# piyanon108/iGate4xSoftphoneDSP

Hardware: AMD Instinct MI355X
Metric: Msamples/s G.711 decode+RMS, 65536ch@8kHz; %HBM roofline at 1/2/4/8 GPU (higher is better)
Workload: dtype u8

## Files before the change

igate4xsoftphonedsp_amd/csrc/igdsp_capi.hip:

```cpp
#include "igdsp_ctx.h"
#include "igdsp_txstage.h"

#include <algorithm>
#include <atomic>
#include <chrono>
#include <cmath>
#include <cstdio>
#include <cstdlib>
#include <cstring>
#include <mutex>
#include <new>
#include <string>
#include <unordered_map>
#include <vector>

using namespace igdsp;
using igdsp_rx::kSlot;
using igdsp_rx::kStageDepth;

struct igdsp_ctx::TxSide {
    igdsp_tx::Stager st;
    hipStream_t stream = nullptr;
    hipEvent_t ev[4] = {};
    igdsp_tx_chan *d_state = nullptr;
// ... 146 lines not shown
    for (int i = 0; i < igdsp_rx::RingMem::kArrays; ++i) if (*ctx->ring.array(i)) (void)hipHostFree(*ctx->ring.array(i));
    const igdsp_rx::Published &p0 = ctx->pub.set(0), &p1 = ctx->pub.set(1);
    void *hosts[] = {ctx->h_up, p0.last, p0.hold, p0.probe, p1.last, p1.hold, p1.probe};
    for (void *p : hosts) if (p) (void)hipHostFree(p);
    void *devs[] = {ctx->d_up, ctx->d_stats, ctx->d_last, ctx->d_hold, ctx->d_probe, ctx->d_queues, ctx->d_enc_tab[0], ctx->d_enc_tab[1]};
    for (void *p : devs) if (p) (void)hipFree(p);
    delete ctx;
    return IGDSP_OK;
}

const char *igdsp_last_error(const igdsp_ctx *ctx) { return ctx ? ctx->err.c_str() : ""; }

int igdsp_device_info(const igdsp_ctx *ctx, int *device, int *compute_units, char *name, size_t name_len)
{
    if (!ctx) return IGDSP_EINVAL;
    if (device) *device = ctx->device;
    if (compute_units) *compute_units = ctx->cus;
    if (name && name_len) { std::strncpy(name, ctx->name.c_str(), name_len - 1); name[name_len - 1] = 0; }
    return IGDSP_OK;
}

int igdsp_set_variant(igdsp_ctx *ctx, int variant)
{
    if (!ctx || variant < 0 || variant > 4) return IGDSP_EINVAL;
    ctx->variant = variant;
    return IGDSP_OK;
}

static uint32_t lookup(igdsp_ctx *ctx, int32_t call_id)
{
    if (call_id >= 0 && call_id < kDirectCalls) return ctx->direct[(size_t)call_id].load(std::memory_order_acquire);
    std::lock_guard<std::mutex> g(ctx->far_mu);
    auto it = ctx->far.find(call_id);
    return it == ctx->far.end() ? kNoChan : it->second;
}

int igdsp_map_call(igdsp_ctx *ctx, int32_t call_id, uint32_t channel)
{
    if (!ctx) return IGDSP_EINVAL;
    if (channel >= ctx->max_channels) return IGDSP_ERANGE;
    if (call_id >= 0 && call_id < kDirectCalls) ctx->direct[(size_t)call_id].store(channel, std::memory_order_release);
    else { std::lock_guard<std::mutex> g(ctx->far_mu); ctx->far[call_id] = channel; }
    return IGDSP_OK;
}

int igdsp_unmap_call(igdsp_ctx *ctx, int32_t call_id)
{
// ... 1034 lines not shown
    if (!ctx || !d_src || !d_dst || (stride & 3u) || n_seg == 0 || (groups && n_items % groups)) return IGDSP_EINVAL;
    HIP_TRY(ctx, hipSetDevice(ctx->device));
    HIP_TRY(ctx, launch_stream_walk(cfg_of(ctx, pick(ctx, stream)), d_src, n_items, stride, hdr, groups, n_seg, trickle, d_dst, d_dst2, pick(ctx, stream)));
    return IGDSP_OK;
}

int igdsp_internal_stream_mix(igdsp_ctx *ctx, const void *d_src, void *d_dst, uint32_t n_items, int r, int w, int waves, void *stream)
{
    if (!ctx || !d_src || !d_dst || (reinterpret_cast<uintptr_t>(d_src) & 3u) || (reinterpret_cast<uintptr_t>(d_dst) & 15u)) return IGDSP_EINVAL;
    HIP_TRY(ctx, hipSetDevice(ctx->device));
    HIP_TRY(ctx, launch_stream_mix(cfg_of(ctx, pick(ctx, stream)), d_src, d_dst, n_items, r, w, waves, pick(ctx, stream)));
    return IGDSP_OK;
}

int igdsp_internal_stream_mix2(igdsp_ctx *ctx, const void *d_src, void *d_dst, void *d_dst2, uint32_t n_items, int r, int w, int waves, void *stream,
                               const void *d_src2)
{
    if (!ctx || !d_src || !d_dst || !d_dst2 || (reinterpret_cast<uintptr_t>(d_src2) & 15u) || ((reinterpret_cast<uintptr_t>(d_src) | reinterpret_cast<uintptr_t>(d_dst) | reinterpret_cast<uintptr_t>(d_dst2)) & 15u)) return IGDSP_EINVAL;
    HIP_TRY(ctx, hipSetDevice(ctx->device));
    HIP_TRY(ctx, launch_stream_mix(cfg_of(ctx, pick(ctx, stream)), d_src, d_dst, n_items, r, w, waves, pick(ctx, stream), d_dst2, d_src2));
    return IGDSP_OK;
}

int igdsp_internal_diag_chunk32(igdsp_ctx *ctx, const uint8_t *d_payload, const uint8_t *d_codec, uint32_t C, uint32_t F,
                                igdsp_frame_stats *d_stats, uint64_t *d_diag, void *stream)
{
    if (!ctx || !d_payload || !d_codec || !d_stats || !d_diag || C < 32) return IGDSP_EINVAL;
    HIP_TRY(ctx, hipSetDevice(ctx->device));
    HIP_TRY(ctx, launch_diag_chunk32(cfg_of(ctx, pick(ctx, stream)), d_payload, d_codec, C, F, d_stats, d_diag, pick(ctx, stream)));
    return IGDSP_OK;
}

int igdsp_dev_alloc(igdsp_ctx *ctx, void **d_ptr, size_t bytes)
{
    if (!ctx || !d_ptr) return IGDSP_EINVAL;
    *d_ptr = nullptr;
    if (bytes == 0) return IGDSP_OK;
    if (hipSetDevice(ctx->device) != hipSuccess) return IGDSP_ENODEV;
    hipError_t e = hipMalloc(d_ptr, bytes);
    return e == hipSuccess ? IGDSP_OK : fail(ctx, IGDSP_ENOMEM, "hipMalloc", e);
}

int igdsp_dev_free(igdsp_ctx *ctx, void *d_ptr)
{
    if (!ctx) return IGDSP_EINVAL;
    if (!d_ptr) return IGDSP_OK;
// ... 128 lines not shown
```

igate4xsoftphonedsp_amd/csrc/igdsp_device.h:

```cpp
#pragma once
#include "igdsp_internal.h"

#include <algorithm>
#include <cstdlib>

namespace igdsp {

__device__ __forceinline__ uint32_t ulaw_abs(uint32_t code)
{
    const uint32_t u = ~code & 0x7Fu;
    return ((((u & 15u) * 2u + 33u) << (u >> 4)) - 33u) << 2;
}

__device__ __forceinline__ uint32_t alaw_abs(uint32_t code)
{
    const uint32_t a = (code ^ 0x55u) & 0x7Fu;
    const uint32_t s = a >> 4, q = a & 15u;
    const uint32_t m = (s == 0u) ? (q * 2u + 1u) : ((q * 2u + 33u) << (s - 1u));
    return m << 3;
}

typedef uint32_t u32x4_t __attribute__((ext_vector_type(4)));
__device__ __forceinline__ uint4 ld_stream(const uint4 *p)
{
// ... 322 lines not shown
    return b >= nb ? b : ((b & 1u) ? half + (b >> 1) : (b >> 1));
}

template <int W>
struct BlockQueue { uint32_t next, batch[8], tag[8]; };

template <int W>
__device__ __forceinline__ void bq_init(BlockQueue<W> &q, uint32_t *gq, uint32_t G, uint32_t gb1)
{
    q.next = (uint32_t)W;
    for (int i = 0; i < 8; ++i) q.tag[i] = 0xFFFFFFFFu;
    q.batch[0] = blockIdx.x; q.tag[0] = 0u;
    q.batch[1] = gq ? gb1 + G : blockIdx.x + G; q.tag[1] = 1u;
}

template <int W>
__device__ __forceinline__ uint32_t bq_grab(BlockQueue<W> &q, uint32_t *gq, uint32_t G, uint32_t lane, uint32_t nb)
{
    uint32_t v = 0;
    if (lane == 0) {
        const uint32_t s = atomicAdd(&q.next, 1u);
        const uint32_t j = s / (uint32_t)W, w = s - j * (uint32_t)W;
        if (w == 0u) {
            const uint32_t nb = gq ? atomicAdd(gq, 1u) + G : blockIdx.x + (j + 1u) * G;
            __hip_atomic_store(&q.batch[(j + 1u) & 7u], nb, __ATOMIC_RELAXED, __HIP_MEMORY_SCOPE_WORKGROUP);
            __hip_atomic_store(&q.tag[(j + 1u) & 7u], j + 1u, __ATOMIC_RELEASE, __HIP_MEMORY_SCOPE_WORKGROUP);
        }
        while (__hip_atomic_load(&q.tag[j & 7u], __ATOMIC_ACQUIRE, __HIP_MEMORY_SCOPE_WORKGROUP) != j)
            __builtin_amdgcn_s_sleep(2);
        v = spread_batch(__hip_atomic_load(&q.batch[j & 7u], __ATOMIC_RELAXED, __HIP_MEMORY_SCOPE_WORKGROUP), nb) * (uint32_t)W + w;
    }
    return (uint32_t)__builtin_amdgcn_readfirstlane((int)v);
}

__device__ __forceinline__ void bq_finish(uint32_t *gq, uint32_t G)
{
    if (gq == nullptr) return;
    __syncthreads();
    if (threadIdx.x == 0 && atomicAdd(gq + 1, 1u) == G - 1u) { gq[0] = 0u; gq[1] = 0u; }
}


struct EncK { int k_and, k_add, sh; uint32_t c_shift, c_seg, base; };

template <int VARIANT>
__device__ __forceinline__ EncK enc_consts(bool alaw)
{
    EncK k;
    if (VARIANT == IGDSP_ENC_SUN16) {
        k.k_and = alaw ? -8 : 0; k.k_add = alaw ? 0 : 0x84; k.sh = 0;
        k.c_shift = alaw ? 23u : 24u;
        k.c_seg = 24u;
    } else {
        k.k_and = alaw ? 0 : 1; k.k_add = alaw ? 0 : 0x21; k.sh = alaw ? 3 : 2;
        k.c_shift = 26u;
        k.c_seg = alaw ? 27u : 26u;
    }
    k.base = alaw ? 0xD5u : 0xFFu;
    return k;
}

template <int VARIANT>
// ... 68 lines not shown
```

igate4xsoftphonedsp_amd/csrc/igdsp_internal.h:

```cpp
#pragma once
#include <hip/hip_runtime.h>
#include <stdint.h>
#include "igdsp.h"
#include "igdsp_route.h"

namespace igdsp {

struct LaunchCfg {
    int compute_units;
    uint32_t *gqueue;
    bool out_spread = false;
    const uint8_t *enc_tab = nullptr;
};

struct WinArgs {
    uint4 *work = nullptr;
    uint32_t gate_mask = 0, alarm = IGDSP_PROBE_ALARM, n_seg = 1, n_groups = 0, F = 0;
    uint32_t gpb = 0, gsh = 0;
    igdsp_chan_hold *hold = nullptr;
    const uint8_t *gate = nullptr;
    igdsp_chan_probe *probe = nullptr;
};
constexpr int kWinRing = 16;
constexpr int kWinBlkCh = 256;
// ... 48 lines not shown
hipError_t launch_conf_copy_ab(const LaunchCfg &cfg, const uint8_t *g711, const uint8_t *codec, const int16_t *pcm, const uint16_t *len,
                               const uint16_t *gain, const uint32_t *port_ptr, const uint32_t *members, uint32_t n_members, uint32_t C, uint32_t P,
                               uint32_t F, uint32_t n, int16_t *out, igdsp_frame_stats *stats, hipStream_t s);
hipError_t launch_bss_select(const LaunchCfg &cfg, const igdsp_rtp_info *info, const uint8_t *g711, const uint8_t *codec, const int16_t *pcm,
                             const uint16_t *len, const uint16_t *gain, const uint32_t *group_ptr, const uint32_t *members, uint32_t n_members,
                             const uint8_t *mute, uint32_t C, uint32_t G, uint32_t F, uint32_t n, uint32_t vote_frames, igdsp_bss_state *state,
                             uint32_t *words, int32_t *sel, int16_t *out, igdsp_frame_stats *stats, hipStream_t s);
hipError_t launch_bss_copy_ab(const LaunchCfg &cfg, const igdsp_rtp_info *info, const uint8_t *g711, const uint8_t *codec, const int16_t *pcm,
                              const uint16_t *len, const uint16_t *gain, const uint32_t *group_ptr, const uint32_t *members, uint32_t n_members,
                              const uint8_t *mute, uint32_t C, uint32_t G, uint32_t F, uint32_t n, uint32_t vote_frames, igdsp_bss_state *state,
                              uint32_t *words, int32_t *sel, int16_t *out, igdsp_frame_stats *stats, hipStream_t s);
hipError_t launch_jb_receive(const LaunchCfg &cfg, const uint8_t *packets, const uint16_t *sizes, const uint8_t *radio, const uint32_t *arrival,
                             uint32_t C, uint32_t T, uint32_t S, uint32_t stride, uint32_t n, uint32_t delay, igdsp_jb_state *state, void *ring,
                             uint8_t *payload, uint16_t *len, igdsp_rtp_info *info, uint8_t *tick, uint8_t *pkt, hipStream_t s);
hipError_t launch_jb_copy(const LaunchCfg &cfg, const uint8_t *packets, const uint16_t *sizes, const uint8_t *radio, const uint32_t *arrival,
                          uint32_t C, uint32_t T, uint32_t S, uint32_t stride, uint32_t n, uint32_t delay, igdsp_jb_state *state, void *ring,
                          uint8_t *payload, uint16_t *len, igdsp_rtp_info *info, uint8_t *tick, uint8_t *pkt, hipStream_t s);
hipError_t launch_wav_expand(const LaunchCfg &cfg, const uint8_t *payload, uint32_t C, uint32_t F, uint32_t n, uint32_t rate,
                             uint8_t *files, uint64_t file_stride, hipStream_t s);
hipError_t launch_g726(const LaunchCfg &cfg, const uint8_t *in, uint8_t *out, uint64_t n_bytes, int mode, hipStream_t s);
hipError_t launch_gen_uniform(uint8_t *out, uint64_t n_bytes, uint64_t seed, uint64_t first_byte, hipStream_t s);
hipError_t launch_stream_rw(const LaunchCfg &cfg, const void *src, size_t bytes, void *dst, hipStream_t s);
hipError_t launch_stream_cluster(const LaunchCfg &cfg, const void *src, size_t bytes, void *dst, int k, hipStream_t s);
hipError_t launch_stream_pieces(const LaunchCfg &cfg, const void *src, uint32_t n_items, uint32_t stride, uint32_t hdr, int mode, int rows, void *dst, void *dst2, hipStream_t s);
hipError_t launch_stream_walk(const LaunchCfg &cfg, const void *src, uint32_t n_items, uint32_t stride, uint32_t hdr, uint32_t groups, uint32_t n_seg,
                              uint32_t trickle, void *dst, void *dst2, hipStream_t s);
hipError_t launch_stream_mix(const LaunchCfg &cfg, const void *src, void *dst, uint32_t n_items, int r, int w, int waves, hipStream_t s, void *dst2 = nullptr, const void *src2 = nullptr);
hipError_t launch_stream_read(const LaunchCfg &cfg, const void *src, size_t bytes, uint64_t *sink, hipStream_t s);

}
```

igate4xsoftphonedsp_amd/csrc/igdsp_k_meter.hip:

```cpp
#include "igdsp_device.h"

namespace igdsp {

__global__ __launch_bounds__(256) void k_meter_wave_per_frame(
    const uint8_t *__restrict__ payload, const uint8_t *__restrict__ codec, const uint16_t *__restrict__ len,
    uint32_t C, uint32_t first_frame, uint32_t n_frames, uint32_t n, igdsp_frame_stats *__restrict__ stats,
    int16_t *__restrict__ pcm, igdsp_aggregate *agg, uint32_t rank)
{
    __shared__ int16_t lut[2][256];
    __shared__ uint2 agg_slots[4 * 4];
    for (uint32_t i = threadIdx.x; i < 512u; i += 256u) {
        const uint32_t code = i & 255u;
        const int ax = (int)((i >> 8) ? alaw_abs(code) : ulaw_abs(code));
        lut[i >> 8][code] = (int16_t)((code & 0x80u) ? ax : -ax);
    }
    __syncthreads();

    const uint32_t lane = threadIdx.x & 63u, wave = threadIdx.x >> 6;
    const bool dword_ok = ((n & 3u) == 0u) && ((reinterpret_cast<uintptr_t>(payload) & 3u) == 0u) &&
                          ((reinterpret_cast<uintptr_t>(pcm) & 7u) == 0u);
    uint64_t a_sumsq = 0, a_samples = 0;
    uint32_t a_frames = 0, a_sil = 0, a_clip = 0, a_bm = 0, a_peak = 0;

    auto load_frame = [&](uint32_t fi) -> uint32_t {
// ... 54 lines not shown
            if (l == 0u) {
                st.sumsq = 0; st.rms = 0.f; st.peak = 0; st.byte_mean = 0; st.flags = IGDSP_FLAG_EMPTY;
            } else {
                st = make_stats(s64, peak, bsum, l, alaw, probe);
                a_sumsq += s64; a_samples += l; a_frames += 1; a_sil += (st.flags & IGDSP_FLAG_SILENT) ? 1u : 0u;
                a_clip += (st.flags & IGDSP_FLAG_CLIPPED) ? 1u : 0u; a_bm += st.byte_mean; a_peak = max(a_peak, peak);
            }
            stats[fi] = st;
        }
    };
    constexpr uint32_t U = 8;
    const uint32_t last = n_frames - 1u;
    for (uint32_t f0 = first_frame + (blockIdx.x * 4u + wave) * U; f0 < n_frames; f0 += gridDim.x * 4u * U) {
        uint32_t w[U];
#pragma unroll
        for (uint32_t u = 0; u < U; ++u) w[u] = load_frame(min(f0 + u, last));
#pragma unroll
        for (uint32_t u = 0; u < U; ++u)
            if (f0 + u < n_frames) process_frame(f0 + u, w[u]);
    }
    if (agg != nullptr) agg_commit_block(agg, rank, agg_slots, 4u, a_sumsq, a_samples, a_frames, a_sil, a_clip, a_bm, a_peak);
}

template <bool STORE_PCM>
__device__ __forceinline__ void process_half(const uint2 *lut, uint2 *strip_half, uint4 (&d)[kLoadsPerChunk],
                                             const uint32_t am, const uint32_t (&fr)[kLoadsPerChunk], const uint32_t (&pm)[kLoadsPerChunk],
                                             const uint32_t off, const uint32_t lane, uint4 *pcm_half, const uint4 *refill,
                                             uint4 *xpose = nullptr)
{
    uint2 e[2][8];
    uint32_t wa[2], wb[2];
    auto issue = [&](int u) {
        const int j = u >> 1, k = u & 1;
        wa[k] = (u & 1) ? d[j].z : d[j].x;
        wb[k] = (u & 1) ? d[j].w : d[j].y;
        const uint32_t lmj = (uint32_t)__builtin_amdgcn_sbfe(am, fr[j], 1) & 0x80808080u;
        const uint32_t ta = (wa[k] & 0x7F7F7F7Fu) | lmj, tb = (wb[k] & 0x7F7F7F7Fu) | lmj;
        e[k][0] = lut_at(lut, ta, off, 0x0C0C0400u); e[k][1] = lut_at(lut, ta, off, 0x0C0C0500u);
        e[k][2] = lut_at(lut, ta, off, 0x0C0C0600u); e[k][3] = lut_at(lut, ta, off, 0x0C0C0700u);
        e[k][4] = lut_at(lut, tb, off, 0x0C0C0400u); e[k][5] = lut_at(lut, tb, off, 0x0C0C0500u);
        e[k][6] = lut_at(lut, tb, off, 0x0C0C0600u); e[k][7] = lut_at(lut, tb, off, 0x0C0C0700u);
    };
    uint32_t sum = 0, peak = 0, bsum = 0;
    uint32_t o[8];
    issue(0);
#pragma unroll
    for (int u = 0; u < 2 * kLoadsPerChunk; ++u) {
        const int j = u >> 1, k = u & 1;
        if (u + 1 < 2 * kLoadsPerChunk) issue(u + 1);
        __builtin_amdgcn_sched_barrier(0);
        bsum = __builtin_amdgcn_sad_u8(wa[k], 0u, bsum);
        bsum = __builtin_amdgcn_sad_u8(wb[k], 0u, bsum);
        sum = sum + e[k][0].x + e[k][1].x; sum = sum + e[k][2].x + e[k][3].x;
        sum = sum + e[k][4].x + e[k][5].x; sum = sum + e[k][6].x + e[k][7].x;
        peak = max(max(peak, e[k][0].y), e[k][1].y); peak = max(max(peak, e[k][2].y), e[k][3].y);
        peak = max(max(peak, e[k][4].y), e[k][5].y); peak = max(max(peak, e[k][6].y), e[k][7].y);
        if (STORE_PCM) {
            o[4 * k + 0] = pack_pcm(wa[k], 0, e[k][0].y, e[k][1].y); o[4 * k + 1] = pack_pcm(wa[k], 2, e[k][2].y, e[k][3].y);
            o[4 * k + 2] = pack_pcm(wb[k], 0, e[k][4].y, e[k][5].y); o[4 * k + 3] = pack_pcm(wb[k], 2, e[k][6].y, e[k][7].y);
        }
        if (k == 1) {
            strip_half[j * 64 + lane] = make_uint2(sum, peak | (bsum << 16) | probe_fail(d[j], pm[j]));
            if (STORE_PCM) {
                const uint32_t wsw = (lane >> 2) & 1u, rsw = lane ^ ((lane >> 3) & 1u);
                xpose[(2u * lane) ^ wsw] = make_uint4(o[0], o[1], o[2], o[3]);
                xpose[(2u * lane + 1u) ^ wsw] = make_uint4(o[4], o[5], o[6], o[7]);
                wave_lds_fence();
                const uint4 v0 = xpose[rsw], v1 = xpose[64u + rsw];
                wave_lds_fence();
                uint4 *op = pcm_half + ((uint32_t)j * 128u + lane);
                op[0] = v0;
                op[64] = v1;
            }
            d[j] = ld_stream(refill + j * 64);
            sum = 0; peak = 0; bsum = 0;
        }
    }
}


template <bool STORE_PCM, bool AGG, bool DIAG = false>
__global__ __launch_bounds__(ChunkGeom<STORE_PCM>::kWaves * 64) void k_meter_chunk64(
    const uint8_t *__restrict__ payload, const uint8_t *__restrict__ codec, uint32_t C, uint32_t n_frames,
    igdsp_frame_stats *__restrict__ stats, int16_t *__restrict__ pcm, igdsp_aggregate *agg, uint32_t rank,
    uint64_t *__restrict__ diag = nullptr, uint32_t *__restrict__ gqueue = nullptr)
{
    constexpr int kWaves = ChunkGeom<STORE_PCM>::kWaves;
    __shared__ uint2 lds[kLutEntries + kWaves * kStripEntries + (STORE_PCM ? kWaves * 256 : 0)];
    constexpr int kRing = 8;
    __shared__ uint32_t q_next, q_batch[kRing], q_tag[kRing];
    __shared__ AggBlock aggb;
    uint64_t d_t0 = 0, d_t1 = 0, d_iter = 0, d_rt0 = 0, d_setup = 0, d_px = 0, d_py = 0, d_red = 0;
    if (DIAG) { d_t0 = now_cycles(); d_rt0 = __builtin_amdgcn_s_memrealtime(); }
    const uint32_t G = gridDim.x;
    uint32_t gb1 = 0;
    if (threadIdx.x == 0 && gqueue != nullptr) gb1 = atomicAdd(gqueue, 1u);
    fill_lut(lds);
    if (threadIdx.x == 0) {
        q_next = kWaves;
        agg_block_init(aggb);
        for (int i = 0; i < kRing; ++i) q_tag[i] = 0xFFFFFFFFu;
        q_batch[0] = blockIdx.x; q_tag[0] = 0u;
        q_batch[1] = gqueue ? gb1 + G : blockIdx.x + G; q_tag[1] = 1u;
    }
    __syncthreads();
    if (DIAG) d_t1 = now_cycles();

    const uint32_t lane = threadIdx.x & 63u, wave = threadIdx.x >> 6;
// ... 87 lines not shown
                if (AGG) {
                    a_sumsq += s << 4; a_bm += bm; a_peak = max(a_peak, peak);
                    u_frames += (uint32_t)kSuperFrames;
                    u_sil += (uint32_t)__builtin_popcountll(__ballot((fl & IGDSP_FLAG_SILENT) != 0u));
                    u_clip += (uint32_t)__builtin_popcountll(__ballot((fl & IGDSP_FLAG_CLIPPED) != 0u));
                }
            }
            wave_lds_fence();
            if (DIAG) { d_iter += 1; d_setup += d_b - d_a; d_px += d_c - d_b; d_py += d_d - d_c; d_red += now_cycles() - d_d; }
            if (!has_next) break;
            sidx = s_next;
            s_next = s_after;
            cur_pt = nxt_pt;
        }
    }
    if (DIAG && lane == 0 && diag != nullptr) {
        uint64_t *o = diag + (uint64_t)(blockIdx.x * kWaves + wave) * 12u;
        o[0] = d_t0; o[1] = d_t1; o[2] = now_cycles(); o[3] = d_setup; o[4] = d_px; o[5] = d_iter; o[6] = d_py;
        o[7] = __builtin_amdgcn_s_getreg((4 << 11) | (0 << 6) | 20);
        o[8] = d_rt0; o[9] = __builtin_amdgcn_s_memrealtime(); o[10] = d_red; o[11] = wave;
    }
    wave_exit(AGG ? agg : nullptr, rank, aggb, (uint32_t)kWaves, lane, gqueue, G, a_sumsq, lane == 0u ? (uint64_t)u_frames * kFrame : 0ull,
              a_bm, a_peak, u_frames, u_sil, u_clip);
}

constexpr int kFatDepth = 4;

template <bool AGG>
__global__ __launch_bounds__(kFatWaves * 64) void k_meter_fat(
    const uint8_t *__restrict__ payload, const uint8_t *__restrict__ codec, uint32_t C, uint32_t n_frames,
    igdsp_frame_stats *__restrict__ stats, igdsp_aggregate *agg, uint32_t rank)
{
    __shared__ uint2 lds[kLutEntries + kFatWaves * kStripEntries];
    fill_lut(lds);
    __syncthreads();

    const uint32_t lane = threadIdx.x & 63u, wave = threadIdx.x >> 6;
    uint2 *strip = lds + kLutEntries + wave * kStripEntries;
    const uint32_t off = (lane & 31u) * 8u;
    uint32_t fr[kLoadsPerChunk], pm[kLoadsPerChunk];
#pragma unroll
    for (int j = 0; j < kLoadsPerChunk; ++j) {
        const uint32_t p = (uint32_t)j * 64u + lane;
        fr[j] = p / 10u;
        pm[j] = probe_mask(p - fr[j] * 10u);
    }
// ... 593 lines not shown
                         reinterpret_cast<const void *>(&k_meter_image<true, false>), reinterpret_cast<const void *>(&k_meter_image<false, false>)};
    for (const void *f : fns) {
        const hipError_t e = hipFuncSetAttribute(f, hipFuncAttributeMaxDynamicSharedMemorySize, lim);
        if (e != hipSuccess) return e;
    }
    return hipSuccess;
}

hipError_t launch_decode_meter(const LaunchCfg &cfg, int variant, const uint8_t *payload, const uint8_t *codec,
                               const uint16_t *len, uint32_t C, uint32_t F, uint32_t n, igdsp_frame_stats *stats,
                               int16_t *pcm, igdsp_aggregate *agg, uint32_t rank, hipStream_t s)
{
    const MeterRoute r = decode_meter_route(C, F, n, variant, len != nullptr, reinterpret_cast<uintptr_t>(payload), reinterpret_cast<uintptr_t>(pcm),
                                            reinterpret_cast<uintptr_t>(stats), (uint32_t)cfg.compute_units, knobs_from_env());
    uint32_t *gq = cfg.gqueue;
    uint64_t *nodiag = nullptr;
    const dim3 g(r.grid), b(r.threads);
    const uint32_t done = r.done, n_frames = C * F;
    with_bool(agg != nullptr, [&](auto A) {
        switch (r.fast) {
        case MeterFast::none: break;
        case MeterFast::fat: hipLaunchKernelGGL((k_meter_fat<A>), g, b, 0, s, payload, codec, C, done, stats, agg, rank); break;
        case MeterFast::chunk:
            with_bool(r.store, [&](auto P) { hipLaunchKernelGGL((k_meter_chunk64<P, A>), g, b, 0, s, payload, codec, C, done, stats, pcm, agg, rank, nodiag, gq); });
            break;
        case MeterFast::tiny:
            with_key(Keys<4, 5, 6, 7, 8>{}, r.key, [&](auto N4) { hipLaunchKernelGGL((k_meter_tiny<N4, A>), g, b, 0, s, payload, codec, C, done, stats, agg, rank, gq); });
            break;
        case MeterFast::strided: {
            auto launch = [&](auto K, auto P) {
                hipLaunchKernelGGL((k_meter_strided<key_q(K), key_tail(K), A, P>), g, b, 0, s, payload, codec, C, done, n, stats, agg, rank, gq, pcm);
            };
            if (r.store) with_key(ReferenceSizeKeys{}, r.key, [&](auto K) { launch(K, std::true_type{}); });
            else         with_key(MeterStridedKeys{}, r.key, [&](auto K) { launch(K, std::false_type{}); });
            break;
        }
        }
    });
    if (r.fast != MeterFast::none) { hipError_t e = hipGetLastError(); if (e != hipSuccess) return e; }
    const dim3 rg(r.rest_grid), rb(r.rest_threads);
    if (r.rest == MeterRest::image) {
        with_bool(agg != nullptr, [&](auto A) { with_bool(len != nullptr, [&](auto L) {
            hipLaunchKernelGGL((k_meter_image<A, L>), rg, rb, r.rest_lds, s, payload, codec, len, C, done, n_frames, n, stats, agg, rank);
        }); });
    } else if (r.rest == MeterRest::wave_per_frame) {
        hipLaunchKernelGGL(k_meter_wave_per_frame, rg, rb, 0, s, payload, codec, len, C, done, n_frames, n, stats, pcm, agg, rank);
    }
// ... 17 lines not shown
```

igate4xsoftphonedsp_amd/csrc/igdsp_k_misc.hip:

```cpp
#include "igdsp_device.h"

namespace igdsp {

constexpr int kWavTile = 16;

__device__ __forceinline__ void wav_header_words(uint32_t (&h)[11], uint32_t rate, uint32_t data_bytes)
{
    h[0] = 0x46464952u;
    h[1] = 36u + data_bytes;
    h[2] = 0x45564157u;
    h[3] = 0x20746D66u;
    h[4] = 16u;
    h[5] = 0x0007u | (2u << 16);
    h[6] = rate;
    h[7] = rate * 4u;
    h[8] = 4u | (16u << 16);
    h[9] = 0x61746164u;
    h[10] = data_bytes;
}

typedef uint32_t u32x4_st4_t __attribute__((ext_vector_type(4), aligned(4)));

__global__ __launch_bounds__(256) void k_wav_expand16(const uint8_t *__restrict__ payload, uint32_t C, uint32_t F, uint32_t n,
                                                      uint32_t rate, uint8_t *__restrict__ files, uint64_t file_stride)
// ... 281 lines not shown
template <int K>
__global__ __launch_bounds__(kBlockThreads) void k_stream_cluster(const uint4 *__restrict__ src, uint32_t n_super, uint4 *__restrict__ dst)
{
    const uint32_t lane = threadIdx.x & 63u, wave = threadIdx.x >> 6;
    const uint32_t n_items = n_super / (uint32_t)K;
    for (uint32_t b = blockIdx.x; b * kWavesPerBlock + wave < n_items; b += gridDim.x) {
        const uint32_t item = b * kWavesPerBlock + wave;
        uint4 acc[K];
#pragma unroll
        for (int k = 0; k < K; ++k) {
            const uint4 *p = src + (((uint64_t)item * (uint32_t)K + (uint32_t)k) * 640u + lane);
            uint4 v[10];
#pragma unroll
            for (int j = 0; j < 10; ++j) v[j] = ld_stream(p + j * 64);
            acc[k] = make_uint4(0, 0, 0, 0);
#pragma unroll
            for (int j = 0; j < 10; ++j) { acc[k].x ^= v[j].x; acc[k].y ^= v[j].y; acc[k].z ^= v[j].z; acc[k].w ^= v[j].w; }
        }
#pragma unroll
        for (int k = 0; k < K; ++k) dst[((uint64_t)item * (uint32_t)K + (uint32_t)k) * 64u + lane] = acc[k];
    }
}

hipError_t launch_stream_cluster(const LaunchCfg &cfg, const void *src, size_t bytes, void *dst, int k, hipStream_t s)
{
    const uint32_t n_super = (uint32_t)(bytes / 10240u);
    const dim3 g(cfg.compute_units), b(kBlockThreads);
    const uint4 *sp = reinterpret_cast<const uint4 *>(src);
    uint4 *dp = reinterpret_cast<uint4 *>(dst);
    if (k == 1) hipLaunchKernelGGL((k_stream_cluster<1>), g, b, 0, s, sp, n_super, dp);
    else if (k == 2) hipLaunchKernelGGL((k_stream_cluster<2>), g, b, 0, s, sp, n_super, dp);
    else if (k == 4) hipLaunchKernelGGL((k_stream_cluster<4>), g, b, 0, s, sp, n_super, dp);
    else if (k == 8) hipLaunchKernelGGL((k_stream_cluster<8>), g, b, 0, s, sp, n_super, dp);
    else if (k == 16) hipLaunchKernelGGL((k_stream_cluster<16>), g, b, 0, s, sp, n_super, dp);
    else return hipErrorInvalidValue;
    return hipGetLastError();
}

hipError_t launch_gen_uniform(uint8_t *out, uint64_t n_bytes, uint64_t seed, uint64_t first_byte, hipStream_t s)
{
    if (n_bytes == 0) return hipSuccess;
    const uint64_t words = (n_bytes >> 3) + 2;
    hipLaunchKernelGGL(k_gen_uniform, dim3(blocks_for(words, 256, 8192)), dim3(256), 0, s, out, n_bytes, seed, first_byte);
    return hipGetLastError();
}

// ... 119 lines not shown
```

igate4xsoftphonedsp_amd/csrc/igdsp_route.h:

```cpp
#pragma once
#include <algorithm>
#include <cstdint>
#include <cstdlib>
#include <optional>
#include <type_traits>
#include <utility>

#include "igdsp.h"

namespace igdsp {


constexpr int kFrame = IGDSP_SAMPLES_PER_FRAME;
constexpr int kChunkFrames = 32;
constexpr int kChunkBytes = kChunkFrames * kFrame;
constexpr int kPiecesPerFrame = kFrame / 16;
constexpr int kPiecesPerChunk = kChunkFrames * kPiecesPerFrame;
constexpr int kLoadsPerChunk = kPiecesPerChunk / 64;
constexpr int kWavesPerBlock = 16;
constexpr int kBlockThreads = kWavesPerBlock * 64;
constexpr int kSuperFrames = 2 * kChunkFrames;
constexpr int kLutEntries = 256 * 32;
constexpr uint32_t kWinMaxSeg = 8;

#ifndef IGDSP_STORE_WAVES
#define IGDSP_STORE_WAVES 4
#endif
template <bool STORE_PCM> struct ChunkGeom { static constexpr int kWaves = STORE_PCM ? IGDSP_STORE_WAVES : kWavesPerBlock; };
constexpr int kFatWaves = 8;
constexpr uint32_t kImgMaxWaves = 12;
#ifndef IGDSP_SSTORE_WAVES
#define IGDSP_SSTORE_WAVES 0
#endif
constexpr int strided_meter_waves(int qp, bool store) { return store ? (IGDSP_SSTORE_WAVES ? IGDSP_SSTORE_WAVES : (qp <= 2 ? 16 : 6)) : (qp <= 11 ? 16 : 12); }
template <int QP, bool STORE = false> struct StridedGeom { static constexpr int kWaves = strided_meter_waves(QP, STORE); };
constexpr int kTinyWaves = 16, kTinyDepth = 4;
#ifndef IGDSP_TINY_SLOT
#define IGDSP_TINY_SLOT 4
#endif
constexpr uint32_t kTinySlot = IGDSP_TINY_SLOT;

#ifndef IGDSP_ENC_WAVES
#define IGDSP_ENC_WAVES 10
#endif
constexpr int kEncWaves = IGDSP_ENC_WAVES;
#ifndef IGDSP_RT_WAVES
#define IGDSP_RT_WAVES 12
#endif
constexpr int kRtWaves = IGDSP_RT_WAVES;
#ifndef IGDSP_RTL_WAVES
#define IGDSP_RTL_WAVES 12
// ... 58 lines not shown
inline uint32_t groups_per_block(uint32_t n_groups, uint32_t cus, std::optional<int> force)
{
    uint32_t gpb = 1u;
    for (uint32_t g = 4u; g > 1u; g >>= 1) if (n_groups % g == 0u && n_groups / g >= cus) { gpb = g; break; }
    if (force) { const uint32_t g = (uint32_t)*force; if ((g == 1u || g == 2u || g == 4u) && n_groups % g == 0u) gpb = g; }
    return gpb;
}
inline uint32_t gpb_shift(uint32_t gpb) { return gpb == 4u ? 2u : (gpb == 2u ? 1u : 0u); }
inline uint32_t rounds_of(uint32_t blocks, uint32_t cus) { return (blocks + cus - 1u) / cus; }

inline bool roundtrip_block_fills(uint32_t blocks, uint32_t cus) { return rounds_of(blocks, cus) == 1u && blocks * 10u >= cus * 6u; }

inline bool window_block_fills(uint32_t blocks, uint32_t cus)
{
    const uint32_t rounds = rounds_of(blocks, cus);
    return rounds == 1u || (uint64_t)blocks * 100u >= (uint64_t)rounds * cus * 85u;
}

enum class MeterFast { none, fat, chunk, tiny, strided };
enum class MeterRest { none, image, wave_per_frame };
struct MeterRoute {
    MeterFast fast = MeterFast::none;
    bool store = false;
    int key = 0;
    uint32_t grid = 0, threads = 0;
    uint32_t done = 0;
    MeterRest rest = MeterRest::none;
    uint32_t rest_grid = 0, rest_threads = 0, rest_lds = 0;
};

inline MeterRoute decode_meter_route(uint32_t C, uint32_t F, uint32_t n, int variant, bool has_len, uintptr_t payload, uintptr_t pcm,
                                     uintptr_t stats, uint32_t cus, const Knobs &k)
{
    MeterRoute r;
    if ((uint64_t)C * F == 0) return r;
    const uint32_t n_frames = C * F;
    const bool chunk_ok = n == (uint32_t)kFrame && !has_len && aligned(payload, 16) && aligned(pcm, 16) && aligned(stats, 16);
    const uint32_t n_super = n_frames / kSuperFrames, whole = n_super * kSuperFrames;
    if (variant == 3 && chunk_ok && pcm == 0 && n_frames >= (uint32_t)kSuperFrames) {
        r.fast = MeterFast::fat;
        r.grid = blocks_for(n_super, kFatWaves, cus); r.threads = kFatWaves * 64; r.done = whole;
    } else if (variant != 1 && chunk_ok && n_frames >= (uint32_t)kSuperFrames) {
        const int w = pcm ? ChunkGeom<true>::kWaves : ChunkGeom<false>::kWaves;
        r.fast = MeterFast::chunk; r.store = pcm != 0;
        r.grid = blocks_for(n_super, w, cus); r.threads = w * 64; r.done = whole;
    }
    if (r.done == 0 && variant != 1 && !has_len && pcm == 0 && (n & 3u) == 0u && n >= 16u && n <= 32u && n_frames >= (uint32_t)kSuperFrames &&
        aligned(payload, 4) && aligned(stats, 16) && !k.no_tiny) {
        r.fast = MeterFast::tiny; r.key = (int)(n >> 2);
        r.grid = blocks_for((n_super + kTinySlot - 1u) / kTinySlot, kTinyWaves, cus); r.threads = kTinyWaves * 64; r.done = whole;
    }
    if (r.done == 0 && variant != 1 && !has_len && (n & 3u) == 0u && n_frames >= (uint32_t)kSuperFrames && ((n >> 2) & 3u) != 3u && n >= 16u &&
        aligned(pcm, 4) && aligned(payload, 4) && aligned(stats, 16) && !k.no_strided) {
        const int key = qt_key(n >> 4, (n & 15u) != 0u);
        if (pcm ? has_key(ReferenceSizeKeys{}, key) : has_key(MeterStridedKeys{}, key)) {
            const int w = strided_meter_waves(key_q(key) + (key_tail(key) ? 1 : 0), pcm != 0);
            r.fast = MeterFast::strided; r.store = pcm != 0; r.key = key;
            r.grid = blocks_for(n_super, w, cus); r.threads = w * 64; r.done = whole;
        }
    }
    if (r.done < n_frames) {
        const bool image_ok = variant != 1 && pcm == 0 && (n & 3u) == 0u && aligned(stats, 16) && aligned(payload, 4) && n_frames - r.done >= 16u;
        if (image_ok) {
            const uint32_t img = (uint32_t)kSuperFrames * n;
            const uint32_t lut_bytes = (uint32_t)kLutEntries * 8u;
            uint32_t waves = std::max(1u, std::min(kImgMaxWaves, (160u * 1024u - lut_bytes - 2048u) / img));
            if (k.img_waves) waves = std::max(1u, std::min(waves, (uint32_t)*k.img_waves));
// ... 257 lines not shown
```

Measured before the change: 5.871 million.

## Split each chunk64 super-frame across a two-wave team with LDS handoff

The no-PCM chunk64 meter kernel now assigns each super-frame to a team of two waves. Each wave decodes half the loads into a double-buffered LDS strip, and one rotating 'folder' wave reduces the per-frame stats and writes them, while the next item is published through a small LDS ring. The aim is more memory-level parallelism and lower per-wave register and latency cost per item, paid for with intra-block spin-wait synchronisation. It also adds a variant 5 that keeps the old one-wave-per-item path, a synthetic streaming 'fronts' probe kernel, and an extra tag wait in bq_grab to fix ring overrun.

```diff
diff --git a/igate4xsoftphonedsp_amd/csrc/igdsp_capi.hip b/igate4xsoftphonedsp_amd/csrc/igdsp_capi.hip
--- a/igate4xsoftphonedsp_amd/csrc/igdsp_capi.hip
+++ b/igate4xsoftphonedsp_amd/csrc/igdsp_capi.hip
@@ -192,7 +192,7 @@
 
 int igdsp_set_variant(igdsp_ctx *ctx, int variant)
 {
-    if (!ctx || variant < 0 || variant > 4) return IGDSP_EINVAL;
+    if (!ctx || variant < 0 || variant > 5) return IGDSP_EINVAL;
     ctx->variant = variant;
     return IGDSP_OK;
 }
@@ -1273,6 +1273,14 @@
     return IGDSP_OK;
 }
 
+int igdsp_internal_stream_fronts(igdsp_ctx *ctx, const void *d_src, void *d_dst, uint32_t *d_queue, uint32_t n_super, int t, int pf, void *stream)
+{
+    if (!ctx || !d_src || !d_dst || !d_queue || ((reinterpret_cast<uintptr_t>(d_src) | reinterpret_cast<uintptr_t>(d_dst)) & 15u)) return IGDSP_EINVAL;
+    HIP_TRY(ctx, hipSetDevice(ctx->device));
+    HIP_TRY(ctx, launch_stream_fronts(cfg_of(ctx, pick(ctx, stream)), d_src, n_super, d_dst, d_queue, t, pf, pick(ctx, stream)));
+    return IGDSP_OK;
+}
+
 int igdsp_internal_diag_chunk32(igdsp_ctx *ctx, const uint8_t *d_payload, const uint8_t *d_codec, uint32_t C, uint32_t F,
                                 igdsp_frame_stats *d_stats, uint64_t *d_diag, void *stream)
 {
diff --git a/igate4xsoftphonedsp_amd/csrc/igdsp_device.h b/igate4xsoftphonedsp_amd/csrc/igdsp_device.h
--- a/igate4xsoftphonedsp_amd/csrc/igdsp_device.h
+++ b/igate4xsoftphonedsp_amd/csrc/igdsp_device.h
@@ -368,6 +368,8 @@
         const uint32_t s = atomicAdd(&q.next, 1u);
         const uint32_t j = s / (uint32_t)W, w = s - j * (uint32_t)W;
         if (w == 0u) {
+            while (__hip_atomic_load(&q.tag[j & 7u], __ATOMIC_ACQUIRE, __HIP_MEMORY_SCOPE_WORKGROUP) != j)
+                __builtin_amdgcn_s_sleep(2);
             const uint32_t nb = gq ? atomicAdd(gq, 1u) + G : blockIdx.x + (j + 1u) * G;
             __hip_atomic_store(&q.batch[(j + 1u) & 7u], nb, __ATOMIC_RELAXED, __HIP_MEMORY_SCOPE_WORKGROUP);
             __hip_atomic_store(&q.tag[(j + 1u) & 7u], j + 1u, __ATOMIC_RELEASE, __HIP_MEMORY_SCOPE_WORKGROUP);
@@ -384,6 +386,49 @@
     if (gq == nullptr) return;
     __syncthreads();
     if (threadIdx.x == 0 && atomicAdd(gq + 1, 1u) == G - 1u) { gq[0] = 0u; gq[1] = 0u; }
+}
+
+template <int T> struct TeamGeom {
+    static_assert(T == 1 || T == 2 || T == 4, "team of 1, 2 or 4 waves");
+    static constexpr int kTeams = kWavesPerBlock / T;
+    static constexpr __host__ __device__ int lo(int r) { return T == 1 ? 0 : T == 2 ? r * kLoadsPerChunk : (r >> 1) * kLoadsPerChunk + (r & 1) * 3; }
+    static constexpr __host__ __device__ int cnt(int r) { return T == 1 ? 2 * kLoadsPerChunk : T == 2 ? kLoadsPerChunk : 3 - (r & 1); }
+};
+struct TeamSync { uint32_t item[4], tag[4], arrive[2], fold[2]; };
+
+__device__ __forceinline__ void team_sync_init(TeamSync &t)
+{
+    for (int i = 0; i < 4; ++i) { t.item[i] = 0xFFFFFFFFu; t.tag[i] = 0xFFFFFFFFu; }
+    t.arrive[0] = t.arrive[1] = 0u; t.fold[0] = t.fold[1] = 0u;
+}
+
+__device__ __forceinline__ void team_signal(uint32_t *ctr, uint32_t lane)
+{
+    __builtin_amdgcn_fence(__ATOMIC_RELEASE, "wavefront");
+    if (lane == 0u) __hip_atomic_fetch_add(ctr, 1u, __ATOMIC_RELAXED, __HIP_MEMORY_SCOPE_WORKGROUP);
+    __builtin_amdgcn_fence(__ATOMIC_ACQUIRE, "wavefront");
+}
+
+__device__ __forceinline__ void team_wait_ge(const uint32_t *ctr, uint32_t v)
+{
+    while (__hip_atomic_load(ctr, __ATOMIC_RELAXED, __HIP_MEMORY_SCOPE_WORKGROUP) < v) __builtin_amdgcn_s_sleep(1);
+    __builtin_amdgcn_fence(__ATOMIC_ACQUIRE, "wavefront");
+}
+
+__device__ __forceinline__ uint32_t team_item(const TeamSync &t, uint32_t k)
+{
+    while (__hip_atomic_load(&t.tag[k & 3u], __ATOMIC_RELAXED, __HIP_MEMORY_SCOPE_WORKGROUP) != k) __builtin_amdgcn_s_sleep(1);
+    __builtin_amdgcn_fence(__ATOMIC_ACQUIRE, "wavefront");
+    return (uint32_t)__builtin_amdgcn_readfirstlane((int)__hip_atomic_load(&t.item[k & 3u], __ATOMIC_RELAXED, __HIP_MEMORY_SCOPE_WORKGROUP));
+}
+
+__device__ __forceinline__ void team_publish(TeamSync &t, uint32_t k, uint32_t id, uint32_t lane)
+{
+    if (lane == 0u) {
+        __hip_atomic_store(&t.item[k & 3u], id, __ATOMIC_RELAXED, __HIP_MEMORY_SCOPE_WORKGROUP);
+        __builtin_amdgcn_fence(__ATOMIC_RELEASE, "wavefront");
+        __hip_atomic_store(&t.tag[k & 3u], k, __ATOMIC_RELAXED, __HIP_MEMORY_SCOPE_WORKGROUP);
+    }
 }
 
 
diff --git a/igate4xsoftphonedsp_amd/csrc/igdsp_internal.h b/igate4xsoftphonedsp_amd/csrc/igdsp_internal.h
--- a/igate4xsoftphonedsp_amd/csrc/igdsp_internal.h
+++ b/igate4xsoftphonedsp_amd/csrc/igdsp_internal.h
@@ -94,6 +94,7 @@
 hipError_t launch_gen_uniform(uint8_t *out, uint64_t n_bytes, uint64_t seed, uint64_t first_byte, hipStream_t s);
 hipError_t launch_stream_rw(const LaunchCfg &cfg, const void *src, size_t bytes, void *dst, hipStream_t s);
 hipError_t launch_stream_cluster(const LaunchCfg &cfg, const void *src, size_t bytes, void *dst, int k, hipStream_t s);
+hipError_t launch_stream_fronts(const LaunchCfg &cfg, const void *src, uint32_t n_super, void *dst, uint32_t *gq, int t, int pf, hipStream_t s);
 hipError_t launch_stream_pieces(const LaunchCfg &cfg, const void *src, uint32_t n_items, uint32_t stride, uint32_t hdr, int mode, int rows, void *dst, void *dst2, hipStream_t s);
 hipError_t launch_stream_walk(const LaunchCfg &cfg, const void *src, uint32_t n_items, uint32_t stride, uint32_t hdr, uint32_t groups, uint32_t n_seg,
                               uint32_t trickle, void *dst, void *dst2, hipStream_t s);
diff --git a/igate4xsoftphonedsp_amd/csrc/igdsp_k_meter.hip b/igate4xsoftphonedsp_amd/csrc/igdsp_k_meter.hip
--- a/igate4xsoftphonedsp_amd/csrc/igdsp_k_meter.hip
+++ b/igate4xsoftphonedsp_amd/csrc/igdsp_k_meter.hip
@@ -100,9 +100,9 @@
     if (agg != nullptr) agg_commit_block(agg, rank, agg_slots, 4u, a_sumsq, a_samples, a_frames, a_sil, a_clip, a_bm, a_peak);
 }
 
-template <bool STORE_PCM>
-__device__ __forceinline__ void process_half(const uint2 *lut, uint2 *strip_half, uint4 (&d)[kLoadsPerChunk],
-                                             const uint32_t am, const uint32_t (&fr)[kLoadsPerChunk], const uint32_t (&pm)[kLoadsPerChunk],
+template <bool STORE_PCM, int N = kLoadsPerChunk>
+__device__ __forceinline__ void process_half(const uint2 *lut, uint2 *strip_half, uint4 (&d)[N],
+                                             const uint32_t am, const uint32_t (&fr)[N], const uint32_t (&pm)[N],
                                              const uint32_t off, const uint32_t lane, uint4 *pcm_half, const uint4 *refill,
                                              uint4 *xpose = nullptr)
 {
@@ -123,9 +123,9 @@
     uint32_t o[8];
     issue(0);
 #pragma unroll
-    for (int u = 0; u < 2 * kLoadsPerChunk; ++u) {
+    for (int u = 0; u < 2 * N; ++u) {
         const int j = u >> 1, k = u & 1;
-        if (u + 1 < 2 * kLoadsPerChunk) issue(u + 1);
+        if (u + 1 < 2 * N) issue(u + 1);
         __builtin_amdgcn_sched_barrier(0);
         bsum = __builtin_amdgcn_sad_u8(wa[k], 0u, bsum);
         bsum = __builtin_amdgcn_sad_u8(wb[k], 0u, bsum);
@@ -157,11 +157,11 @@
 }
 
 
-template <bool STORE_PCM, bool AGG, bool DIAG = false>
-__global__ __launch_bounds__(ChunkGeom<STORE_PCM>::kWaves * 64) void k_meter_chunk64(
+template <bool STORE_PCM, bool AGG, bool DIAG>
+__device__ __forceinline__ void chunk64_wave_body(
     const uint8_t *__restrict__ payload, const uint8_t *__restrict__ codec, uint32_t C, uint32_t n_frames,
     igdsp_frame_stats *__restrict__ stats, int16_t *__restrict__ pcm, igdsp_aggregate *agg, uint32_t rank,
-    uint64_t *__restrict__ diag = nullptr, uint32_t *__restrict__ gqueue = nullptr)
+    uint64_t *__restrict__ diag, uint32_t *__restrict__ gqueue)
 {
     constexpr int kWaves = ChunkGeom<STORE_PCM>::kWaves;
     __shared__ uint2 lds[kLutEntries + kWaves * kStripEntries + (STORE_PCM ? kWaves * 256 : 0)];
@@ -295,6 +295,154 @@
     }
     wave_exit(AGG ? agg : nullptr, rank, aggb, (uint32_t)kWaves, lane, gqueue, G, a_sumsq, lane == 0u ? (uint64_t)u_frames * kFrame : 0ull,
               a_bm, a_peak, u_frames, u_sil, u_clip);
+}
+
+template <int NP, bool AGG, bool DIAG>
+__device__ __forceinline__ void chunk64_team_wave(
+    const uint8_t *__restrict__ payload, const uint8_t *__restrict__ codec, uint32_t C, uint32_t n_super,
+    igdsp_frame_stats *__restrict__ stats, const uint2 *lut, uint2 *strips, TeamSync &ts, BlockQueue<kWavesPerBlock> &q,
+    uint32_t *__restrict__ gqueue, uint32_t n_batches, uint32_t team, uint32_t trank, uint32_t lane, uint64_t (&dg)[5],
+    uint64_t &a_sumsq, uint32_t &a_bm, uint32_t &a_peak, uint32_t &u_frames, uint32_t &u_sil, uint32_t &u_clip)
+{
+    constexpr uint32_t T = kTeamWaves;
+    const uint32_t G = gridDim.x;
+    const int lo = TeamGeom<kTeamWaves>::lo((int)trank);
+    const uint32_t half = (uint32_t)lo / (uint32_t)kLoadsPerChunk, j0 = (uint32_t)lo % (uint32_t)kLoadsPerChunk;
+    const uint32_t pofs = half * (uint32_t)kPiecesPerChunk + j0 * 64u;
+    const uint32_t off = (lane & 31u) * 8u;
+    uint32_t fr[NP], pm[NP];
+#pragma unroll
+    for (int i = 0; i < NP; ++i) {
+        const uint32_t p = (j0 + (uint32_t)i) * 64u + lane;
+        fr[i] = p / 10u;
+        pm[i] = probe_mask(p - fr[i] * 10u);
+    }
+    const uint4 *src16 = reinterpret_cast<const uint4 *>(payload);
+    auto fetch_pt = [&](uint32_t sidx) { return (uint32_t)codec[(sidx * (uint32_t)kSuperFrames + lane) % C]; };
+    auto grab = [&]() { return bq_grab<kWavesPerBlock>(q, gqueue, G, lane, n_batches); };
+
+    uint32_t cur = spread_batch(blockIdx.x, n_batches) * (uint32_t)kWavesPerBlock + team;
+    if (trank == 0u) team_publish(ts, 1u, cur < n_super ? grab() : 0xFFFFFFFFu, lane);
+    if (cur >= n_super) return;
+    uint32_t cur_pt = fetch_pt(cur);
+    uint4 d[NP];
+#pragma unroll
+    for (int i = 0; i < NP; ++i) d[i] = ld_stream(src16 + ((uint64_t)cur * (uint32_t)kStripEntries + pofs + (uint32_t)i * 64u + lane));
+    for (uint32_t k = 0;; ++k) {
+        const uint32_t b = k & 1u, u = k >> 1;
+        const bool folder = trank == k % T;
+        const uint32_t nxt = team_item(ts, k + 1u);
+        if (folder) team_publish(ts, k + 2u, nxt < n_super ? grab() : 0xFFFFFFFFu, lane);
+        const uint32_t s_load = nxt < n_super ? nxt : 0u;
+        const bool my_alaw = cur_pt == IGDSP_PT_PCMA;
+        const uint64_t amask = __ballot(my_alaw);
+        const uint32_t am = half ? (uint32_t)(amask >> 32) : (uint32_t)amask;
+        const uint4 *nsrc = src16 + ((uint64_t)s_load * (uint32_t)kStripEntries + pofs + lane);
+        const uint32_t nxt_pt = fetch_pt(s_load);
+        uint2 *strip = strips + b * (uint32_t)kStripEntries;
+        uint64_t t0 = 0, t1 = 0, t2 = 0;
+        if (DIAG) t0 = now_cycles();
+        team_wait_ge(&ts.fold[b], u);
+        if (DIAG) t1 = now_cycles();
+        process_half<false, NP>(lut, strip + pofs, d, am, fr, pm, off, lane, nullptr, nsrc);
+        team_signal(&ts.arrive[b], lane);
+        if (DIAG) { t2 = now_cycles(); dg[0] += t1 - t0; dg[1] += t2 - t1; dg[2] += 1; }
+        if (folder) {
+            team_wait_ge(&ts.arrive[b], T * (u + 1u));
+            uint64_t t3 = 0;
+            if (DIAG) { t3 = now_cycles(); dg[3] += t3 - t2; }
+            const uint4 *row = reinterpret_cast<const uint4 *>(strip + lane * kPiecesPerFrame);
+            uint64_t s = 0;
+            uint32_t peak = 0, bsum = 0, fail = 0;
+#pragma unroll
+            for (int i = 0; i < kPiecesPerFrame / 2; ++i) {
+                const uint4 v = row[i];
+                s += (uint64_t)(v.x + v.z);
+                peak = max(max(peak, v.y & 0x7FFFu), v.w & 0x7FFFu);
+                bsum += ((v.y >> 16) & 0x7FFFu) + ((v.w >> 16) & 0x7FFFu);
+                fail |= v.y | v.w;
+            }
+            team_signal(&ts.fold[b], lane);
+            uint32_t bm, fl;
+            st_stream(reinterpret_cast<uint4 *>(stats + (cur * (uint32_t)kSuperFrames + lane)), pack_stats160(s, peak, bsum, my_alaw, (fail >> 31) == 0u, bm, fl));
+            if (AGG) {
+                a_sumsq += s << 4; a_bm += bm; a_peak = max(a_peak, peak);
+                u_frames += (uint32_t)kSuperFrames;
+                u_sil += (uint32_t)__builtin_popcountll(__ballot((fl & IGDSP_FLAG_SILENT) != 0u));
+                u_clip += (uint32_t)__builtin_popcountll(__ballot((fl & IGDSP_FLAG_CLIPPED) != 0u));
+            }
+            if (DIAG) dg[4] += now_cycles() - t3;
+        }
+        if (nxt >= n_super) break;
+        cur = nxt;
+        cur_pt = nxt_pt;
+    }
+}
+
+template <bool AGG, bool DIAG>
+__device__ __forceinline__ void chunk64_team_body(
+    const uint8_t *__restrict__ payload, const uint8_t *__restrict__ codec, uint32_t C, uint32_t n_frames,
+    igdsp_frame_stats *__restrict__ stats, igdsp_aggregate *agg, uint32_t rank, uint64_t *__restrict__ diag, uint32_t *__restrict__ gqueue)
+{
+    using TG = TeamGeom<kTeamWaves>;
+    __shared__ uint2 lds[kLutEntries + TG::kTeams * 2 * kStripEntries];
+    __shared__ BlockQueue<kWavesPerBlock> q;
+    __shared__ TeamSync ts[TG::kTeams];
+    __shared__ AggBlock aggb;
+    uint64_t d_t0 = 0, d_t1 = 0, d_rt0 = 0;
+    if (DIAG) { d_t0 = now_cycles(); d_rt0 = __builtin_amdgcn_s_memrealtime(); }
+    const uint32_t G = gridDim.x;
+    uint32_t gb1 = 0;
+    if (threadIdx.x == 0 && gqueue != nullptr) gb1 = atomicAdd(gqueue, 1u);
+    fill_lut(lds);
+    if (threadIdx.x == 0) {
+        bq_init<kWavesPerBlock>(q, gqueue, G, gb1);
+        q.next = (uint32_t)TG::kTeams;
+        agg_block_init(aggb);
+    }
+    if (threadIdx.x < (uint32_t)TG::kTeams) team_sync_init(ts[threadIdx.x]);
+    __syncthreads();
+    if (DIAG) d_t1 = now_cycles();
+
+    const uint32_t lane = threadIdx.x & 63u, wave = threadIdx.x >> 6, team = wave / (uint32_t)kTeamWaves, trank = wave % (uint32_t)kTeamWaves;
+    const uint32_t n_batches = IGDSP_SPREAD_METER ? (n_frames / kSuperFrames + (uint32_t)kWavesPerBlock - 1u) / (uint32_t)kWavesPerBlock : 0u;
+    const uint32_t n_super = n_frames / kSuperFrames;
+    uint2 *strips = lds + kLutEntries + team * 2u * (uint32_t)kStripEntries;
+    uint64_t a_sumsq = 0;
+    uint32_t a_bm = 0, a_peak = 0, u_frames = 0, u_sil = 0, u_clip = 0;
+    uint64_t dg[5] = {0, 0, 0, 0, 0};
+    if ((trank & 1u) == 0u)
+        chunk64_team_wave<TG::cnt(0), AGG, DIAG>(payload, codec, C, n_super, stats, lds, strips, ts[team], q, gqueue, n_batches, team, trank, lane, dg,
+                                        a_sumsq, a_bm, a_peak, u_frames, u_sil, u_clip);
+    else
+        chunk64_team_wave<TG::cnt(1), AGG, DIAG>(payload, codec, C, n_super, stats, lds, strips, ts[team], q, gqueue, n_batches, team, trank, lane, dg,
+                                        a_sumsq, a_bm, a_peak, u_frames, u_sil, u_clip);
+    if (DIAG && lane == 0 && diag != nullptr) {
+        uint64_t *o = diag + (uint64_t)(blockIdx.x * kWavesPerBlock + wave) * 12u;
+        o[0] = d_t0; o[1] = d_t1; o[2] = now_cycles(); o[3] = dg[0]; o[4] = dg[1]; o[5] = dg[2]; o[6] = dg[3];
+        o[7] = __builtin_amdgcn_s_getreg((4 << 11) | (0 << 6) | 20);
+        o[8] = d_rt0; o[9] = __builtin_amdgcn_s_memrealtime(); o[10] = dg[4]; o[11] = wave;
+    }
+    wave_exit(AGG ? agg : nullptr, rank, aggb, (uint32_t)kWavesPerBlock, lane, gqueue, G, a_sumsq, lane == 0u ? (uint64_t)u_frames * kFrame : 0ull,
+              a_bm, a_peak, u_frames, u_sil, u_clip);
+}
+
+template <bool STORE_PCM, bool AGG, bool DIAG = false>
+__global__ __launch_bounds__(ChunkGeom<STORE_PCM>::kWaves * 64) void k_meter_chunk64(
+    const uint8_t *__restrict__ payload, const uint8_t *__restrict__ codec, uint32_t C, uint32_t n_frames,
+    igdsp_frame_stats *__restrict__ stats, int16_t *__restrict__ pcm, igdsp_aggregate *agg, uint32_t rank,
+    uint64_t *__restrict__ diag = nullptr, uint32_t *__restrict__ gqueue = nullptr)
+{
+    if constexpr (STORE_PCM) chunk64_wave_body<true, AGG, DIAG>(payload, codec, C, n_frames, stats, pcm, agg, rank, diag, gqueue);
+    else chunk64_team_body<AGG, DIAG>(payload, codec, C, n_frames, stats, agg, rank, diag, gqueue);
+}
+
+template <bool AGG>
+__global__ __launch_bounds__(kWavesPerBlock * 64) void k_meter_chunk64_wave(
+    const uint8_t *__restrict__ payload, const uint8_t *__restrict__ codec, uint32_t C, uint32_t n_frames,
+    igdsp_frame_stats *__restrict__ stats, igdsp_aggregate *agg, uint32_t rank, uint32_t *__restrict__ gqueue)
+{
+    chunk64_wave_body<false, AGG, false>(payload, codec, C, n_frames, stats, nullptr, agg, rank, nullptr, gqueue);
 }
 
 constexpr int kFatDepth = 4;
@@ -934,7 +1082,8 @@
         case MeterFast::none: break;
         case MeterFast::fat: hipLaunchKernelGGL((k_meter_fat<A>), g, b, 0, s, payload, codec, C, done, stats, agg, rank); break;
         case MeterFast::chunk:
-            with_bool(r.store, [&](auto P) { hipLaunchKernelGGL((k_meter_chunk64<P, A>), g, b, 0, s, payload, codec, C, done, stats, pcm, agg, rank, nodiag, gq); });
+            if (r.waves_own) hipLaunchKernelGGL((k_meter_chunk64_wave<A>), g, b, 0, s, payload, codec, C, done, stats, agg, rank, gq);
+            else with_bool(r.store, [&](auto P) { hipLaunchKernelGGL((k_meter_chunk64<P, A>), g, b, 0, s, payload, codec, C, done, stats, pcm, agg, rank, nodiag, gq); });
             break;
         case MeterFast::tiny:
             with_key(Keys<4, 5, 6, 7, 8>{}, r.key, [&](auto N4) { hipLaunchKernelGGL((k_meter_tiny<N4, A>), g, b, 0, s, payload, codec, C, done, stats, agg, rank, gq); });
diff --git a/igate4xsoftphonedsp_amd/csrc/igdsp_k_misc.hip b/igate4xsoftphonedsp_amd/csrc/igdsp_k_misc.hip
--- a/igate4xsoftphonedsp_amd/csrc/igdsp_k_misc.hip
+++ b/igate4xsoftphonedsp_amd/csrc/igdsp_k_misc.hip
@@ -327,6 +327,88 @@
     }
 }
 
+template <int T, bool PF, int NP>
+__device__ __forceinline__ void fronts_wave(const uint4 *__restrict__ src, uint32_t n_super, uint4 *__restrict__ dst, uint32_t *gq,
+                                            BlockQueue<kWavesPerBlock> &q, TeamSync &ts, uint4 *strip, uint32_t rank, uint32_t lane,
+                                            uint32_t cur)
+{
+    const uint32_t G = gridDim.x;
+    const int lo = TeamGeom<T>::lo((int)rank);
+    if (rank == 0u) team_publish(ts, 1u, cur < n_super ? bq_grab<kWavesPerBlock>(q, gq, G, lane, 0u) : 0xFFFFFFFFu, lane);
+    uint4 v[NP];
+    if (PF && cur < n_super) {
+#pragma unroll
+        for (int i = 0; i < NP; ++i) v[i] = ld_stream(src + ((uint64_t)cur * 640u + (uint32_t)(lo + i) * 64u + lane));
+    }
+    for (uint32_t k = 0; cur < n_super; ++k) {
+        const uint32_t b = k & 1u, u = k >> 1;
+        const bool mine = rank == k % (uint32_t)T;
+        const uint32_t nxt = team_item(ts, k + 1u);
+        if (mine) team_publish(ts, k + 2u, nxt < n_super ? bq_grab<kWavesPerBlock>(q, gq, G, lane, 0u) : 0xFFFFFFFFu, lane);
+        const uint32_t ld = nxt < n_super ? nxt : cur;
+        uint4 acc = make_uint4(rank == 0u ? cur : 0u, rank == 0u ? lane : 0u, 0u, 0u);
+        if (!PF) {
+#pragma unroll
+            for (int i = 0; i < NP; ++i) v[i] = ld_stream(src + ((uint64_t)cur * 640u + (uint32_t)(lo + i) * 64u + lane));
+        }
+        uint4 *sb = strip + b * (uint32_t)(T * 64);
+        team_wait_ge(&ts.fold[b], u);
+#pragma unroll
+        for (int i = 0; i < NP; ++i) { acc.x ^= v[i].x; acc.y ^= v[i].y; acc.z ^= v[i].z; acc.w ^= v[i].w; }
+        sb[rank * 64u + lane] = acc;
+        if (PF) {
+            __builtin_amdgcn_sched_barrier(0);
+#pragma unroll
+            for (int i = 0; i < NP; ++i) v[i] = ld_stream(src + ((uint64_t)ld * 640u + (uint32_t)(lo + i) * 64u + lane));
+        }
+        team_signal(&ts.arrive[b], lane);
+        if (mine) {
+            team_wait_ge(&ts.arrive[b], (uint32_t)T * (u + 1u));
+            uint4 x = sb[lane];
+#pragma unroll
+            for (int r = 1; r < T; ++r) { const uint4 y = sb[r * 64 + lane]; x.x ^= y.x; x.y ^= y.y; x.z ^= y.z; x.w ^= y.w; }
+            team_signal(&ts.fold[b], lane);
+            st_stream(dst + ((uint64_t)cur * 64u + lane), x);
+        }
+        cur = nxt;
+    }
+}
+
+template <int T, bool PF>
+__global__ __launch_bounds__(kBlockThreads) void k_stream_fronts(const uint4 *__restrict__ src, uint32_t n_super, uint4 *__restrict__ dst, uint32_t *gq)
+{
+    using TG = TeamGeom<T>;
+    __shared__ BlockQueue<kWavesPerBlock> q;
+    __shared__ TeamSync ts[TG::kTeams];
+    __shared__ uint4 strip[TG::kTeams * 2 * T * 64];
+    uint32_t gb1 = 0;
+    if (threadIdx.x == 0) {
+        gb1 = gq ? atomicAdd(gq, 1u) : 0u;
+        bq_init<kWavesPerBlock>(q, gq, gridDim.x, gb1);
+        q.next = (uint32_t)TG::kTeams;
+    }
+    if (threadIdx.x < (uint32_t)TG::kTeams) team_sync_init(ts[threadIdx.x]);
+    __syncthreads();
+    const uint32_t lane = threadIdx.x & 63u, wave = threadIdx.x >> 6, team = wave / (uint32_t)T, rank = wave % (uint32_t)T;
+    const uint32_t cur = blockIdx.x * (uint32_t)kWavesPerBlock + team;
+    uint4 *st = strip + team * (uint32_t)(2 * T * 64);
+    if (TG::cnt((int)rank) == 3) fronts_wave<T, PF, (T == 4 ? 3 : TG::cnt(0))>(src, n_super, dst, gq, q, ts[team], st, rank, lane, cur);
+    else fronts_wave<T, PF, (T == 4 ? 2 : TG::cnt(0))>(src, n_super, dst, gq, q, ts[team], st, rank, lane, cur);
+    bq_finish(gq, gridDim.x);
+}
+
+hipError_t launch_stream_fronts(const LaunchCfg &cfg, const void *src, uint32_t n_super, void *dst, uint32_t *gq, int t, int pf, hipStream_t s)
+{
+    if (n_super == 0) return hipSuccess;
+    const dim3 g(cfg.compute_units), b(kBlockThreads);
+    const uint4 *sp = reinterpret_cast<const uint4 *>(src);
+    uint4 *dp = reinterpret_cast<uint4 *>(dst);
+#define IGDSP_FRONTS(T_, PF_) if (t == T_ && (pf != 0) == PF_) { hipLaunchKernelGGL((k_stream_fronts<T_, PF_>), g, b, 0, s, sp, n_super, dp, gq); return hipGetLastError(); }
+    IGDSP_FRONTS(1, false) IGDSP_FRONTS(1, true) IGDSP_FRONTS(2, false) IGDSP_FRONTS(2, true) IGDSP_FRONTS(4, false) IGDSP_FRONTS(4, true)
+#undef IGDSP_FRONTS
+    return hipErrorInvalidValue;
+}
+
 hipError_t launch_stream_cluster(const LaunchCfg &cfg, const void *src, size_t bytes, void *dst, int k, hipStream_t s)
 {
     const uint32_t n_super = (uint32_t)(bytes / 10240u);
diff --git a/igate4xsoftphonedsp_amd/csrc/igdsp_route.h b/igate4xsoftphonedsp_amd/csrc/igdsp_route.h
--- a/igate4xsoftphonedsp_amd/csrc/igdsp_route.h
+++ b/igate4xsoftphonedsp_amd/csrc/igdsp_route.h
@@ -27,6 +27,7 @@
 #define IGDSP_STORE_WAVES 4
 #endif
 template <bool STORE_PCM> struct ChunkGeom { static constexpr int kWaves = STORE_PCM ? IGDSP_STORE_WAVES : kWavesPerBlock; };
+constexpr int kTeamWaves = 2;
 constexpr int kFatWaves = 8;
 constexpr uint32_t kImgMaxWaves = 12;
 #ifndef IGDSP_SSTORE_WAVES
@@ -131,6 +132,7 @@
 struct MeterRoute {
     MeterFast fast = MeterFast::none;
     bool store = false;
+    bool waves_own = false;
     int key = 0;
     uint32_t grid = 0, threads = 0;
     uint32_t done = 0;
@@ -151,7 +153,7 @@
         r.grid = blocks_for(n_super, kFatWaves, cus); r.threads = kFatWaves * 64; r.done = whole;
     } else if (variant != 1 && chunk_ok && n_frames >= (uint32_t)kSuperFrames) {
         const int w = pcm ? ChunkGeom<true>::kWaves : ChunkGeom<false>::kWaves;
-        r.fast = MeterFast::chunk; r.store = pcm != 0;
+        r.fast = MeterFast::chunk; r.store = pcm != 0; r.waves_own = variant == 5 && pcm == 0;
         r.grid = blocks_for(n_super, w, cus); r.threads = w * 64; r.done = whole;
     }
     if (r.done == 0 && variant != 1 && !has_len && pcm == 0 && (n & 3u) == 0u && n >= 16u && n <= 32u && n_frames >= (uint32_t)kSuperFrames &&
```

Result: no change. 5.926 million (median of 6 runs) (+0.9%).
